# alexeygrigorev/kubernetes-deep-learning

Measured on AMD Instinct MI355X. Metric: images/sec (whole node) + p50 latency, Xception 299x299 at 1/2/4/8 MI355X, higher is better.
Workload: dtype bf16; 1 GPU; model=Keras Xception 299x299 + clothing head (21,067,390 params), global_batch=32, image_size=299, per_gpu_batch=32, parallelism=dp1, ingress=local, egress=local, hipgraph=True, lanes=1, stages=2 (cut after block8_sepconv3)

## Files before the change

kdl/csrc/bindings_gpu.cpp:

```cpp
#include <pybind11/pybind11.h>
#include <pybind11/stl.h>

#include "kernels/launch.h"
#include "runtime/jpeg_huff.h"
#include "runtime/engine.h"
#include "runtime/comm.h"
#include "runtime/dp_hiploop.h"
#include "runtime/hip_backend.h"

namespace py = pybind11;
using namespace kdl;

namespace {

template <typename T>
T* P(const py::dict& d, const char* k) {
  if (!d.contains(k) || d[k].is_none()) return nullptr;
  return reinterpret_cast<T*>(d[k].cast<uintptr_t>());
}
int I(const py::dict& d, const char* k, int def = 0) {
  if (!d.contains(k) || d[k].is_none()) return def;
  return d[k].cast<int>();
}
hipStream_t S(uintptr_t s) { return reinterpret_cast<hipStream_t>(s); }

ConvGemmArgs conv_args(const py::dict& d) {
  ConvGemmArgs a{};
  a.x = P<const uint16_t>(d, "x");
  a.wp = P<const uint16_t>(d, "wp");
  a.bias = P<const float>(d, "bias");
  a.dww = P<const float>(d, "dww");
  a.dwk = P<const uint16_t>(d, "dwk");
  a.res = P<const uint16_t>(d, "res");
  a.y = P<uint16_t>(d, "y");
  a.stamps = P<unsigned long long>(d, "stamps");
  a.B = I(d, "B"); a.H = I(d, "H"); a.W = I(d, "W");
  a.OH = I(d, "OH"); a.OW = I(d, "OW"); a.M = I(d, "M");
  a.ldx = I(d, "ldx"); a.ldy = I(d, "ldy"); a.ldr = I(d, "ldr");
  a.K = I(d, "K"); a.cin = I(d, "cin", 32); a.NF = I(d, "NF");
  a.nstore = I(d, "nstore"); a.stride = I(d, "stride", 1);
  a.relu_in = I(d, "relu_in"); a.relu_out = I(d, "relu_out"); a.opad = I(d, "opad");
  a.dt = I(d, "dt");
  a.krot = I(d, "krot");
  a.ksplit = I(d, "ksplit");
  a.ws = P<float>(d, "ws");
  a.cnt = P<int>(d, "cnt");
  a.ascale = P<const float>(d, "ascale");
  a.ascale_ld = I(d, "ascale_ld");
  return a;
}
float F(const py::dict& d, const char* k, float def) {
  if (!d.contains(k) || d[k].is_none()) return def;
  return d[k].cast<float>();
}
StemArgs stem_args(const py::dict& d) {
  StemArgs a{};
  a.x = P<const void>(d, "x"); a.wp = P<const uint16_t>(d, "wp");
  a.bias = P<const float>(d, "bias"); a.y = P<uint16_t>(d, "y");
  a.B = I(d, "B"); a.H = I(d, "H"); a.W = I(d, "W");
  a.OH = I(d, "OH"); a.OW = I(d, "OW"); a.ldy = I(d, "ldy"); a.in_kind = I(d, "in_kind");
  a.KH = I(d, "KH", 3); a.KW = I(d, "KW", 3); a.stride = I(d, "stride", 2); a.pad = I(d, "pad", 0);
  a.cout = I(d, "cout", 32); a.relu = I(d, "relu", 1); a.dt = I(d, "dt");
  const char* sk[3] = {"scale0", "scale1", "scale2"};
  const char* hk[3] = {"shift0", "shift1", "shift2"};
  for (int c = 0; c < 3; ++c) { a.scale[c] = F(d, sk[c], 1.f); a.shift[c] = F(d, hk[c], 0.f); }
  a.rows = I(d, "rows", 0);
  return a;
}
GapArgs gap_args(const py::dict& d) {
  GapArgs a{};
  a.x = P<const uint16_t>(d, "x"); a.y = P<float>(d, "y"); a.yb = P<uint16_t>(d, "yb");
  a.B = I(d, "B"); a.HW = I(d, "HW"); a.ldx = I(d, "ldx"); a.F = I(d, "F"); a.dt = I(d, "dt");
  return a;
}
FcArgs fc_args(const py::dict& d) {
  FcArgs a{};
  a.x = P<const float>(d, "x"); a.w = P<const float>(d, "w"); a.bias = P<const float>(d, "bias");
  a.out = P<float>(d, "out");
  a.B = I(d, "B"); a.F = I(d, "F"); a.N = I(d, "N"); a.relu = I(d, "relu");
  return a;
}
PatchifyArgs patch_args(const py::dict& d) {
  PatchifyArgs a{};
  a.x = P<const uint8_t>(d, "x"); a.y = P<uint16_t>(d, "y");
  a.B = I(d, "B"); a.H = I(d, "H"); a.W = I(d, "W"); a.P = I(d, "P"); a.ldy = I(d, "ldy");
  const char* sk[3] = {"scale0", "scale1", "scale2"};
  const char* hk[3] = {"shift0", "shift1", "shift2"};
  for (int c = 0; c < 3; ++c) { a.scale[c] = F(d, sk[c], 1.f); a.shift[c] = F(d, hk[c], 0.f); }
  return a;
}
EmbedArgs embed_args(const py::dict& d) {
  EmbedArgs a{};
  a.x = P<uint16_t>(d, "x"); a.cls = P<const float>(d, "cls"); a.pos = P<const float>(d, "pos");
  a.B = I(d, "B"); a.T = I(d, "T"); a.D = I(d, "D");
  return a;
}
LnArgs ln_args(const py::dict& d) {
  LnArgs a{};
  a.x = P<const uint16_t>(d, "x"); a.y = P<uint16_t>(d, "y");
  a.gamma = P<const float>(d, "gamma"); a.beta = P<const float>(d, "beta");
  a.y8 = P<uint8_t>(d, "y8"); a.inv_scale = F(d, "inv_scale", 1.f);
  a.rows = d["rows"].cast<long>(); a.D = I(d, "D"); a.ldx = I(d, "ldx"); a.ldy = I(d, "ldy");
  a.eps = F(d, "eps", 1e-6f);
  return a;
}
AttnArgs attn_args(const py::dict& d) {
  AttnArgs a{};
  a.qkv = P<const uint16_t>(d, "qkv"); a.out = P<uint16_t>(d, "out");
  a.out8 = P<uint8_t>(d, "out8"); a.inv_scale = F(d, "inv_scale", 1.f);
  a.B = I(d, "B"); a.T = I(d, "T"); a.H = I(d, "H"); a.dh = I(d, "dh", 64);
  a.scale = F(d, "scale", 0.125f);
  return a;
}
DwkArgs dwk_args(const py::dict& d) {
  DwkArgs a{};
  a.x = P<const uint16_t>(d, "x"); a.w = P<const float>(d, "w"); a.bias = P<const float>(d, "bias");
  a.y = P<uint16_t>(d, "y"); a.pool = P<float>(d, "pool"); a.w1 = P<const float>(d, "w1");
  a.B = I(d, "B"); a.H = I(d, "H"); a.W = I(d, "W"); a.C = I(d, "C"); a.OH = I(d, "OH"); a.OW = I(d, "OW");
  a.K = I(d, "K"); a.S = I(d, "S", 1); a.pad = I(d, "pad"); a.act = I(d, "act"); a.Cs = I(d, "Cs");
  a.cg = I(d, "cg", 0); a.rb = I(d, "rb", 0); a.tw = I(d, "tw", 0); a.seg = I(d, "seg", 0);
  a.lds_kb = I(d, "lds_kb", 0); a.algo = I(d, "algo", 0); a.pd = I(d, "pd", 0);
// ... 98 lines not shown
}
ResampleArgs resample_args(const py::dict& d) {
  ResampleArgs a{};
  a.desc = P<const ResampleDesc>(d, "desc"); a.h_desc = P<const ResampleDesc>(d, "h_desc");
  a.jdesc = P<const JpegDesc>(d, "jdesc"); a.h_jdesc = P<const JpegDesc>(d, "h_jdesc");
  a.planes = P<const uint8_t>(d, "planes"); a.tmp = P<uint8_t>(d, "tmp"); a.out = P<uint8_t>(d, "out");
  a.plane_cap = U64(d, "plane_cap"); a.tmp_cap = U64(d, "tmp_cap");
  a.n_jdesc = I(d, "n_jdesc"); a.n = I(d, "n"); a.out_rows = I(d, "out_rows");
  a.OH = I(d, "OH"); a.OW = I(d, "OW");
  return a;
}

DwArgs dw_args(const py::dict& d) {
  DwArgs a{};
  a.x = P<const uint16_t>(d, "x"); a.w = P<const float>(d, "w"); a.y = P<uint16_t>(d, "y");
  a.B = I(d, "B"); a.H = I(d, "H"); a.W = I(d, "W"); a.C = I(d, "C"); a.relu_in = I(d, "relu_in");
  a.cg = d.contains("cg") ? I(d, "cg") : 0; a.rb = d.contains("rb") ? I(d, "rb") : 0;
  a.tw = d.contains("tw") ? I(d, "tw") : 0; a.seg = d.contains("seg") ? I(d, "seg") : 0;
  a.algo = d.contains("algo") ? I(d, "algo") : 0; a.pd = d.contains("pd") ? I(d, "pd") : 0;
  return a;
}

void chk(hipError_t e, const char* what) { check_hip(e, what); }

}

PYBIND11_MODULE(_C, m) {
  m.doc() = "kdl MI355X (gfx950) HIP kernels and native executor";

  m.def("conv_gemm", [](int mode, int cfg, py::dict d, uintptr_t s) {
    const auto a = conv_args(d);
    py::gil_scoped_release nogil;
    chk(conv_gemm(mode, cfg, a, S(s)), "conv_gemm");
  });
  m.def("conv_gemm_config", [](int cfg) {
    int bm = 0, bn = 0, th = 0;
    if (conv_gemm_config(cfg, &bm, &bn, &th) != 0) throw std::out_of_range("bad conv_gemm config");
    return py::make_tuple(bm, bn, th);
  });
  m.def("conv_gemm_num_configs", &conv_gemm_num_configs);
  m.def("memcpy_async", [](uintptr_t dst, uintptr_t src, size_t n, int kind, uintptr_t s) {
    py::gil_scoped_release nogil;
    chk(hipMemcpyAsync((void*)dst, (const void*)src, n, (hipMemcpyKind)kind, S(s)), "memcpy_async");
  });
  m.def("dw3x3", [](py::dict d, uintptr_t s) {
    const auto a = dw_args(d);
    py::gil_scoped_release nogil;
    chk(dw3x3(a, S(s)), "dw3x3");
  });
  m.def("stem_conv", [](py::dict d, uintptr_t s) {
    const auto a = stem_args(d);
    py::gil_scoped_release nogil;
    chk(stem_conv(a, S(s)), "stem_conv");
  });
  m.def("pool_add", [](py::dict d, uintptr_t s) {
    const auto a = pool_args(d);
    py::gil_scoped_release nogil;
    chk(pool_add(a, S(s)), "pool_add");
  });
  m.def("head_dense", [](py::dict d, uintptr_t s) {
    const auto a = head_args(d);
    py::gil_scoped_release nogil;
    chk(head_dense(a, S(s)), "head_dense");
  });
  m.def("gap", [](py::dict d, uintptr_t s) {
    const auto a = gap_args(d);
    py::gil_scoped_release nogil;
    chk(gap(a, S(s)), "gap");
  });
  m.def("fc", [](py::dict d, uintptr_t s) {
    const auto a = fc_args(d);
    py::gil_scoped_release nogil;
    chk(fc(a, S(s)), "fc");
  });
  m.def("patchify", [](py::dict d, uintptr_t s) {
    const auto a = patch_args(d);
    py::gil_scoped_release nogil;
    chk(patchify(a, S(s)), "patchify");
  });
  m.def("embed_tokens", [](py::dict d, uintptr_t s) {
    const auto a = embed_args(d);
    py::gil_scoped_release nogil;
    chk(embed_tokens(a, S(s)), "embed_tokens");
  });
  m.def("layernorm", [](py::dict d, uintptr_t s) {
    const auto a = ln_args(d);
    py::gil_scoped_release nogil;
    chk(layernorm(a, S(s)), "layernorm");
  });
  m.def("attention", [](py::dict d, uintptr_t s) {
    const auto a = attn_args(d);
    py::gil_scoped_release nogil;
    chk(attention(a, S(s)), "attention");
  });
  m.def("dwk", [](py::dict d, uintptr_t s) {
    const auto a = dwk_args(d);
    py::gil_scoped_release nogil;
    chk(dwk(a, S(s)), "dwk");
  });
  m.def("dwk_tiles", [](py::dict d) {
    const auto a = dwk_args(d);
    int cg, rb, tw, nt;
    dwk_tiles(a, &cg, &rb, &tw, &nt);
    return py::make_tuple(cg, rb, tw, nt, dwk_seg(a));
  });
  m.def("squeeze_excite", [](py::dict d, uintptr_t s) {
// ... 194 lines not shown
  py::class_<HLLeader>(m, "HipLoopDpLeader")
      .def(py::init([](HipExecBackend* be, loop::Comm* sc, loop::Comm* ga, std::vector<int> buckets, double timeout_s,
                       double ping_s) {
             auto h = new HLLeader();
             h->local = std::make_unique<HipLoopLocal>(be);
             h->lead = std::make_unique<HipLoopDpLeader>(h->local.get(), sc, ga, std::move(buckets), timeout_s, ping_s);
             return h;
           }),
           py::arg("local"), py::arg("scatter"), py::arg("gather"), py::arg("rank_buckets"), py::arg("timeout_s") = 120.0,
           py::arg("ping_s") = 0.0, py::keep_alive<1, 2>(), py::keep_alive<1, 3>(), py::keep_alive<1, 4>())
      .def("api_ptr", [](const HLLeader& l) { return reinterpret_cast<uintptr_t>(l.lead->api()); })
      .def_property_readonly("world", [](const HLLeader& l) { return l.lead->world(); })
      .def_property_readonly("steps", [](const HLLeader& l) { return l.lead->steps(); })
      .def_property_readonly("broken", [](const HLLeader& l) { return l.lead->broken(); })
      .def("send_ctrl", [](HLLeader& l, int cmd, int version) {
        py::gil_scoped_release nogil;
        return l.lead->send_ctrl(cmd, version);
      })
      .def("ping", [](HLLeader& l) {
        py::gil_scoped_release nogil;
        return l.lead->ping();
      });
  py::class_<HLFollower>(m, "HipLoopDpFollower")
      .def(py::init([](HipExecBackend* be, loop::Comm* sc, loop::Comm* ga) {
             auto h = new HLFollower();
             h->local = std::make_unique<HipLoopLocal>(be);
             h->f = std::make_unique<HipLoopDpFollower>(h->local.get(), sc, ga);
             return h;
           }),
           py::keep_alive<1, 2>(), py::keep_alive<1, 3>(), py::keep_alive<1, 4>())
      .def_property_readonly("steps", [](const HLFollower& f) { return f.f->steps(); })
      .def("run", [](HLFollower& f, double liveness_s) {
        DpCtrl c{};
        {
          py::gil_scoped_release nogil;
          c = f.f->run(liveness_s);
        }
        return std::make_tuple(c.cmd, c.version, c.seq);
      }, py::arg("liveness_s") = 30.0);
  m.attr("DP_STOP") = int(DP_STOP);
  m.attr("DP_BATCH") = int(DP_BATCH);
  m.attr("DP_RELOAD") = int(DP_RELOAD);
  m.attr("DP_PING") = int(DP_PING);

  py::class_<Program>(m, "Program")
      .def(py::init<>())
      .def("add_conv_gemm", [](Program& p, const std::string& name, int mode, int cfg, py::dict d) {
        Op op; op.kind = OP_CONV_GEMM; op.name = name; op.mode = mode; op.cfg = cfg; op.g = conv_args(d);
        p.add(op);
      })
      .def("add_stem", [](Program& p, const std::string& name, py::dict d) {
        Op op; op.kind = OP_STEM; op.name = name; op.st = stem_args(d); p.add(op);
      })
      .def("add_pool_add", [](Program& p, const std::string& name, py::dict d) {
        Op op; op.kind = OP_POOL_ADD; op.name = name; op.pa = pool_args(d); p.add(op);
      })
      .def("add_head", [](Program& p, const std::string& name, py::dict d) {
        Op op; op.kind = OP_HEAD; op.name = name; op.hd = head_args(d); p.add(op);
      })
      .def("add_gap", [](Program& p, const std::string& name, py::dict d) {
        Op op; op.kind = OP_GAP; op.name = name; op.gp = gap_args(d); p.add(op);
      })
      .def("add_fc", [](Program& p, const std::string& name, py::dict d) {
        Op op; op.kind = OP_FC; op.name = name; op.fc = fc_args(d); p.add(op);
      })
      .def("add_patchify", [](Program& p, const std::string& name, py::dict d) {
        Op op; op.kind = OP_PATCHIFY; op.name = name; op.pt = patch_args(d); p.add(op);
      })
      .def("add_embed", [](Program& p, const std::string& name, py::dict d) {
        Op op; op.kind = OP_EMBED; op.name = name; op.em = embed_args(d); p.add(op);
      })
      .def("add_layernorm", [](Program& p, const std::string& name, py::dict d) {
        Op op; op.kind = OP_LN; op.name = name; op.ln = ln_args(d); p.add(op);
      })
      .def("add_attention", [](Program& p, const std::string& name, py::dict d) {
        Op op; op.kind = OP_ATTN; op.name = name; op.at = attn_args(d); p.add(op);
      })
      .def("add_dwk", [](Program& p, const std::string& name, py::dict d) {
        Op op; op.kind = OP_DWK; op.name = name; op.dk = dwk_args(d); p.add(op);
      })
      .def("add_se", [](Program& p, const std::string& name, py::dict d) {
        Op op; op.kind = OP_SE; op.name = name; op.se = se_args(d); p.add(op);
      })
      .def("add_chscale", [](Program& p, const std::string& name, py::dict d) {
        Op op; op.kind = OP_CHSCALE; op.name = name; op.cs = chs_args(d); p.add(op);
      })
      .def("add_entry_block", [](Program& p, const std::string& name, int cfg, py::dict d) {
        Op op; op.kind = OP_ENTRY_BLOCK; op.name = name; op.cfg = cfg; op.eb = eb_args(d); p.add(op);
      })
      .def("add_gemm_f8", [](Program& p, const std::string& name, int cfg, py::dict d) {
        Op op; op.kind = OP_GEMM_F8; op.name = name; op.cfg = cfg; op.f8 = f8_args(d); p.add(op);
      })
      .def("add_fc_mfma", [](Program& p, const std::string& name, py::dict d) {
        Op op; op.kind = OP_FC_MFMA; op.name = name; op.fcm = fcm_args(d); p.add(op);
      })
      .def("add_resize", [](Program& p, const std::string& name, py::dict d) {
        Op op; op.kind = OP_RESIZE; op.name = name; op.rs = resize_args(d); p.add(op);
      })
      .def("add_dw", [](Program& p, const std::string& name, py::dict d) {
        Op op; op.kind = OP_DW; op.name = name; op.dw = dw_args(d); p.add(op);
      })
      .def("add_memset", [](Program& p, const std::string& name, uintptr_t ptr, size_t bytes) {
        Op op; op.kind = OP_MEMSET; op.name = name; op.mem_ptr = reinterpret_cast<void*>(ptr);
        op.mem_bytes = bytes; p.add(op);
      })
      .def("set_cfg", [](Program& p, size_t i, int cfg) { p.mutable_op(i).cfg = cfg; })
// ... 18 lines not shown
```

kdl/csrc/kernels/launch.h:

```cpp
#pragma once
#include <hip/hip_runtime.h>
#include <stdint.h>

namespace kdl {

struct ConvGemmArgs {
  const uint16_t* x;
  const uint16_t* wp;
  const float* bias;
  const float* dww;
  const uint16_t* dwk;
  const uint16_t* res;
  uint16_t* y;
  int B, H, W;
  int OH, OW;
  int M;
  int ldx, ldy, ldr;
  int K;
  int cin;
  int NF;
  int nstore;
  int stride;
  int relu_in;
  int relu_out;
// ... 29 lines not shown
  const uint16_t* wr;
  const float* br;
  int B, H, W, OH, OW, ldx, ldy;
  int grid;
  const int4* steps;
  const int* step_off;
  unsigned long long* stamps;
};
hipError_t entry_block(int cfg, const EntryBlockArgs& a, hipStream_t s);
int entry_block_config(int cfg, int* c0, int* c1, int* pc, int* lds, int* occ);

constexpr int C3_CFG_BASE = 208;
hipError_t conv3x3_2d(int cfg, const ConvGemmArgs& a, hipStream_t s);
int conv3x3_2d_config(int cfg, int* bm, int* bn, int* threads);
constexpr int S2D_CFG_BASE = 160;
hipError_t sepconv_2d(int cfg, const ConvGemmArgs& a, hipStream_t s);
int sepconv_2d_config(int cfg, int* bm, int* bn, int* threads);
constexpr int STREAM_CFG_BASE = 3000;
hipError_t gemm_stream(const ConvGemmArgs& a, bool nt, hipStream_t s);
bool gemm_stream_shape(int K, int nstore, int dt = 0);
hipError_t conv_gemm(int mode, int cfg, const ConvGemmArgs& a, hipStream_t s);
hipError_t gemm_pipe(int mode, int cfg, const ConvGemmArgs& a, hipStream_t s);
int gemm_pipe_config(int cfg, int* bm, int* bn, int* threads);
int conv_gemm_config(int cfg, int* bm, int* bn, int* threads);
int conv_gemm_num_configs();

struct DwArgs {
  const uint16_t* x;
  const float* w;
  uint16_t* y;
  int B, H, W, C;
  int relu_in;
  int cg, rb, tw, seg;
  int algo;
  int pd;
};
hipError_t dw3x3(const DwArgs& a, hipStream_t s);

struct StemArgs {
  const void* x;
  const uint16_t* wp;
  const float* bias;
  uint16_t* y;
  int B, H, W, OH, OW, ldy;
  int in_kind;
  int KH, KW, stride, pad, cout;
  float scale[3], shift[3];
  int relu;
  int dt;
  int rows;
};
hipError_t stem_conv(const StemArgs& a, hipStream_t s);

struct PoolAddArgs {
  const uint16_t* x;
  const uint16_t* res;
  uint16_t* y;
  int B, H, W, OH, OW, C;
  int pad_top, pad_left;
  int dt;
  int algo;
  int seg, rb;
};
hipError_t pool_add(const PoolAddArgs& a, hipStream_t s);

struct GapArgs {
  const uint16_t* x;
  float* y;
  uint16_t* yb;
  int B, HW, ldx, F;
  int dt;
};
hipError_t gap(const GapArgs& a, hipStream_t s);

struct FcArgs {
  const float* x;
  const float* w;
  const float* bias;
  float* out;
  int B, F, N, relu;
};
hipError_t fc(const FcArgs& a, hipStream_t s);

struct FcMfmaArgs {
  const uint16_t* xb;
  const uint16_t* wp;
  const float* bias;
  float* out;
  int B, F, N, NF, relu;
  int dt;
};
hipError_t fc_mfma(const FcMfmaArgs& a, hipStream_t s);

struct PatchifyArgs {
  const uint8_t* x;
  uint16_t* y;
  int B, H, W, P, ldy;
  float scale[3], shift[3];
};
hipError_t patchify(const PatchifyArgs& a, hipStream_t s);

struct EmbedArgs {
  uint16_t* x;
  const float* cls;
  const float* pos;
  int B, T, D;
// ... 149 lines not shown
```

kdl/csrc/runtime/engine.cpp:

```cpp
#include "engine.h"

#include <algorithm>

namespace kdl {

void check_hip(hipError_t e, const std::string& what) {
  if (e != hipSuccess) throw std::runtime_error(what + ": " + hipGetErrorString(e));
}

hipError_t run_op(const Op& op, hipStream_t s) {
  switch (op.kind) {
    case OP_CONV_GEMM: return conv_gemm(op.mode, op.cfg, op.g, s);
    case OP_STEM: return stem_conv(op.st, s);
    case OP_POOL_ADD: return pool_add(op.pa, s);
    case OP_HEAD: return head_dense(op.hd, s);
    case OP_RESIZE: return resize_nearest_u8(op.rs, s);
    case OP_MEMSET: return hipMemsetAsync(op.mem_ptr, 0, op.mem_bytes, s);
    case OP_DW: return dw3x3(op.dw, s);
    case OP_GAP: return gap(op.gp, s);
    case OP_FC: return fc(op.fc, s);
    case OP_FC_MFMA: return fc_mfma(op.fcm, s);
    case OP_PATCHIFY: return patchify(op.pt, s);
    case OP_EMBED: return embed_tokens(op.em, s);
    case OP_LN: return layernorm(op.ln, s);
    case OP_ATTN: return attention(op.at, s);
    case OP_DWK: return dwk(op.dk, s);
    case OP_SE: return squeeze_excite(op.se, s);
    case OP_CHSCALE: return channel_scale(op.cs, s);
    case OP_GEMM_F8: return gemm_f8(op.cfg, op.f8, s);
    case OP_ENTRY_BLOCK: return entry_block(op.cfg, op.eb, s);
  }
  return hipErrorInvalidValue;
}

Program::~Program() { reset(); }

void Program::reset() {
  if (exec_) (void)hipGraphExecDestroy(exec_);
  if (graph_) (void)hipGraphDestroy(graph_);
  exec_ = nullptr;
  graph_ = nullptr;
}

void Program::run(hipStream_t s) const {
  for (const auto& op : ops_) check_hip(run_op(op, s), "launch " + op.name);
}

void Program::capture(hipStream_t s) {
  reset();
  check_hip(hipStreamBeginCapture(s, hipStreamCaptureModeThreadLocal), "hipStreamBeginCapture");
  hipError_t err = hipSuccess;
  std::string bad;
  for (const auto& op : ops_) {
    err = run_op(op, s);
    if (err != hipSuccess) { bad = op.name; break; }
  }
  hipGraph_t g = nullptr;
  const hipError_t e2 = hipStreamEndCapture(s, &g);
  if (err != hipSuccess) {
    if (g) (void)hipGraphDestroy(g);
    check_hip(err, "capture launch " + bad);
  }
  check_hip(e2, "hipStreamEndCapture");
  graph_ = g;
  check_hip(hipGraphInstantiate(&exec_, graph_, nullptr, nullptr, 0), "hipGraphInstantiate");
}

void Program::launch(hipStream_t s) const {
  if (exec_) check_hip(hipGraphLaunch(exec_, s), "hipGraphLaunch");
  else run(s);
}

std::vector<float> Program::profile(hipStream_t s, int iters) const {
  const size_t n = ops_.size();
  std::vector<hipEvent_t> ev(n + 1);
  for (auto& e : ev) check_hip(hipEventCreate(&e), "hipEventCreate");
  std::vector<std::vector<float>> t(n);
  for (int it = 0; it < iters; ++it) {
    check_hip(hipEventRecord(ev[0], s), "record");
    for (size_t i = 0; i < n; ++i) {
      check_hip(run_op(ops_[i], s), "launch " + ops_[i].name);
      check_hip(hipEventRecord(ev[i + 1], s), "record");
    }
// ... 20 lines not shown
```

kdl/csrc/runtime/engine.h:

```cpp
#pragma once
#include <hip/hip_runtime.h>

#include <stdexcept>
#include <string>
#include <vector>

#include "../kernels/launch.h"

namespace kdl {

enum OpKind { OP_CONV_GEMM = 0, OP_STEM = 1, OP_POOL_ADD = 2, OP_HEAD = 3, OP_RESIZE = 4, OP_MEMSET = 5, OP_DW = 6, OP_GAP = 7, OP_FC = 8, OP_FC_MFMA = 9,
              OP_PATCHIFY = 10, OP_EMBED = 11, OP_LN = 12, OP_ATTN = 13,
              OP_DWK = 14, OP_SE = 15, OP_CHSCALE = 16, OP_GEMM_F8 = 17,
              OP_ENTRY_BLOCK = 21 };

struct Op {
  OpKind kind;
  std::string name;
  int mode = 0, cfg = 0;
  ConvGemmArgs g{};
  StemArgs st{};
  PoolAddArgs pa{};
  HeadArgs hd{};
  ResizeArgs rs{};
  DwArgs dw{};
  GapArgs gp{};
  FcArgs fc{};
  FcMfmaArgs fcm{};
  PatchifyArgs pt{};
  EmbedArgs em{};
  LnArgs ln{};
  AttnArgs at{};
  DwkArgs dk{};
  SeArgs se{};
  ChScaleArgs cs{};
  GemmF8Args f8{};
  EntryBlockArgs eb{};
  void* mem_ptr = nullptr;
  size_t mem_bytes = 0;
};

void check_hip(hipError_t e, const std::string& what);

hipError_t run_op(const Op& op, hipStream_t s);

class Program {
 public:
  Program() = default;
  ~Program();
  Program(const Program&) = delete;
  Program& operator=(const Program&) = delete;

  void add(const Op& op) {
    if (exec_) throw std::runtime_error("Program already captured; reset() first");
    ops_.push_back(op);
  }
  size_t size() const { return ops_.size(); }
  const Op& op(size_t i) const { return ops_.at(i); }
  Op& mutable_op(size_t i) { return ops_.at(i); }

  void run(hipStream_t s) const;
  void capture(hipStream_t s);
  void launch(hipStream_t s) const;
  bool captured() const { return exec_ != nullptr; }
  void reset();
  std::vector<float> profile(hipStream_t s, int iters) const;

 private:
  std::vector<Op> ops_;
  hipGraph_t graph_ = nullptr;
  hipGraphExec_t exec_ = nullptr;
};

}
```

kdl/engine/xception.py:

```python
from __future__ import annotations

import os
from pathlib import Path

import torch

from ..models import xception as X
from ..models.layers import tf_same_pad
from ..ops import _lib
from ..ops.conv import MODE_CONV, MODE_DW, MODE_PW, ConvGemmLayer, Geometry, conv_weights_nk
from ..ops.pack import bn_scale_shift, pack_fragments, round_up, rowrun_weights
from .base import EngineBase, Step


class XceptionEngine(EngineBase):
    model_name = "xception"

    def __init__(self, params: dict, max_batch: int = 32, device: str | torch.device = "cuda",
                 in_kind: str = "u8", head: X.Head = X.DEFAULT_HEAD, buckets=None,
                 tune_file: str | Path | None = None):
        super().__init__(device, max_batch, buckets)
        self.in_kind = in_kind
        self.head = head
        eb = os.environ.get("KDL_ENTRY_BLOCK", "2:15,3")
        spec = "2,3" if eb == "1" else ("" if eb == "0" else eb)
        self.fused_blocks = {}
        for v in filter(None, (x.strip() for x in spec.split(","))):
            blk, _, cfg = v.partition(":")
            self.fused_blocks[int(blk)] = int(cfg) if cfg else None
        self.size = X.INPUT_SIZE
        self.shapes: dict[str, tuple[int, int, int]] = {}
        self._build(params)
        self._alloc()
        if tune_file and Path(tune_file).exists():
            self.load_tuning(tune_file)

    def _build(self, p: dict) -> None:
        dev = self.device
        S = self.size
        st = X.SPEC
        c1 = st[0].main[0]
        s, t = bn_scale_shift(p, c1.bn)
        w = p[f"{c1.name}/kernel"].double().reshape(27, 32).t() * s[:, None]
        if self.in_kind == "u8":
            bias = t - w.sum(1)
            w = w / 127.5
        else:
            bias = t
        oh1 = (S - 3) // 2 + 1
        self.stem_rows = self.in_kind == "u8" and os.environ.get("KDL_STEM_ROWS", "1") != "0"
        if self.stem_rows:
            self.stem_wp = pack_fragments(rowrun_weights(w, 3, 9, 16), 2, 2).to(dev).contiguous()
        else:
            self.stem_wp = pack_fragments(w, 2, 1).to(dev).contiguous()
        self.stem_bias = bias.float().to(dev)
        self.steps.append(Step("stem", c1.name, src="input", dst="stem1", geom=(S, S, oh1, oh1)))
        self.shapes["stem1"] = (oh1, oh1, 32)
        c2 = st[0].main[1]
        s, t = bn_scale_shift(p, c2.bn)
        w = conv_weights_nk(p[f"{c2.name}/kernel"], 32) * s[:, None]
        lay = ConvGemmLayer(c2.name, MODE_CONV, w, t, cin_pad=32, n=64, relu_out=True, device=dev)
        h = oh1 - 2
        self.steps.append(Step("conv", c2.name, lay, "stem1", "stem2", geom=(oh1, oh1, h, h)))
        self.shapes["stem2"] = (h, h, 64)
        cur, H = "stem2", h
        for bi, blk in enumerate(st[1:], start=1):
            if blk.kind in ("entry", "exit"):
                rc = blk.res_conv
                oh = (H - 1) // 2 + 1
                rname = f"{rc.name}_out"
                lay = self._pw(p, rc, dev)
                _, pt, _ = tf_same_pad(H, 3, 2)
                out = f"block{bi + 1}_out"
                if bi + 1 in self.fused_blocks:
                    from ..ops.entry_block import EntryBlock
                    s1, s2 = (self._sep(p, op, dev) for op in blk.main)
                    g = os.environ.get("KDL_ENTRY_GRID")
                    fb = EntryBlock(f"block{bi + 1}", s1, s2, lay, cfg=self.fused_blocks[bi + 1], device=dev,
                                    grid=int(g) if g else None)
                    self.steps.append(Step("block", f"block{bi + 1}", src=cur, dst=out, geom=(H, H, oh, oh),
                                           extra=dict(eb=fb)))
                    self.shapes[out] = (oh, oh, s2.ldy)
                    cur, H = out, oh
                    continue
                self.steps.append(Step("conv", rc.name, lay, cur, rname, geom=(H, H, oh, oh)))
                self.shapes[rname] = (oh, oh, lay.ldy)
                y = cur
                for op in blk.main:
                    lay = self._sep(p, op, dev)
                    dst = f"{op.name}_out"
                    self.steps.append(Step("conv", op.name, lay, y, dst, geom=(H, H, H, H)))
                    self.shapes[dst] = (H, H, lay.ldy)
                    y = dst
                C = self.shapes[y][2]
                self.steps.append(Step("pool", f"block{bi + 1}_pool", src=y, dst=out, res=rname,
                                       geom=(H, H, oh, oh), extra=dict(pad=pt, C=C)))
                self.shapes[out] = (oh, oh, C)
                cur, H = out, oh
            elif blk.kind == "middle":
                y = cur
                for k, op in enumerate(blk.main):
                    lay = self._sep(p, op, dev)
                    dst = f"{op.name}_out"
                    res = cur if k == len(blk.main) - 1 else None
                    self.steps.append(Step("conv", op.name, lay, y, dst, res=res, geom=(H, H, H, H)))
                    self.shapes[dst] = (H, H, lay.ldy)
                    y = dst
                cur = y
            else:
                for op in blk.main:
                    lay = self._sep(p, op, dev)
                    dst = f"{op.name}_out"
                    self.steps.append(Step("conv", op.name, lay, cur, dst, geom=(H, H, H, H)))
                    self.shapes[dst] = (H, H, lay.ldy)
                    cur = dst
        hd = self.head
# ... 15 lines not shown
            if (a.kind == "conv" and b.kind == "conv" and b.src == a.dst and uses.get(a.dst) == 1
                    and a.res is None and a.layer.relu_out == 0 and b.layer.mode == MODE_DW and b.layer.relu_in):
                a.layer.relu_out, b.layer.relu_in = 1, False

    @staticmethod
    def _pw(p, rc, dev) -> ConvGemmLayer:
        s, t = bn_scale_shift(p, rc.bn)
        cin_pad = round_up(rc.cin, 32)
        w = torch.zeros(rc.cout, cin_pad, dtype=torch.float64)
        w[:, :rc.cin] = p[f"{rc.name}/kernel"].double()[0, 0].t() * s[:, None]
        return ConvGemmLayer(rc.name, MODE_PW, w, t, cin_pad=cin_pad, n=rc.cout, stride=2, device=dev)

    @staticmethod
    def _sep(p, op, dev) -> ConvGemmLayer:
        s, t = bn_scale_shift(p, op.bn)
        cin_pad = round_up(op.cin, 32)
        w = torch.zeros(op.cout, cin_pad, dtype=torch.float64)
        w[:, :op.cin] = p[f"{op.name}/pointwise_kernel"].double()[0, 0].t() * s[:, None]
        dww = torch.zeros(9, cin_pad, dtype=torch.float32)
        dww[:, :op.cin] = p[f"{op.name}/depthwise_kernel"].float()[:, :, :, 0].reshape(9, op.cin)
        return ConvGemmLayer(op.name, MODE_DW, w, t, cin_pad=cin_pad, n=op.cout, dww=dww,
                             relu_in=op.relu_in, relu_out=op.relu_out, device=dev,
                             ksplit=(2, 3, 4) if op.cout >= 1536 else ())

    def _alloc(self) -> None:
        B, S, dev = self.max_batch, self.size, self.device
        if self.in_kind == "u8":
            self.inp = torch.zeros((B, S, S, 3), dtype=torch.uint8, device=dev)
        else:
            self.inp = torch.zeros((B, S, S, 3), dtype=torch.float32, device=dev)
        self.bufs: dict[str, torch.Tensor] = {}
        for name, (h, w, c) in self.shapes.items():
            self.bufs[name] = torch.zeros(B * h * w * c, dtype=torch.bfloat16, device=dev)
        self.logits = torch.zeros((B, self.head.classes), dtype=torch.float32, device=dev)
        self.head_feat = torch.zeros((B, self.head.features), dtype=torch.float32, device=dev)
        self.head_hid = torch.zeros((self.head.features // 64, B, self.head.hidden_units), dtype=torch.float32,
                                    device=dev)
        n = 1
        for st in self.conv_steps():
            if st.layer.mode == MODE_DW:
                H, W, _, _ = st.geom
                n = max(n, B * H * W * st.layer.cin_pad)
        self.dwtmp = torch.zeros(n, dtype=torch.bfloat16, device=dev)
        self.bufs["__dwtmp"] = self.dwtmp

    def _ptr(self, name: str) -> int:
        if name == "input":
            return self.input_ptr()
        if name == "logits":
            return self.output_ptr()
        return _lib.ptr(self.bufs[self._remap.get(name, name)])


    def scratch_buffers(self) -> list[str]:
        return ["__dwtmp"]

    def _emit(self, prog, step: Step, b: int) -> None:
        H, W, OH, OW = step.geom
        if step.kind == "stem":
            prog.add_stem(step.name, dict(x=self.input_ptr(), wp=_lib.ptr(self.stem_wp),
                                          bias=_lib.ptr(self.stem_bias), y=self._ptr(step.dst),
                                          B=b, H=H, W=W, OH=OH, OW=OW, ldy=32,
                                          in_kind=0 if self.in_kind == "u8" else 1, rows=int(self.stem_rows)))
        elif step.kind == "conv":
            self._emit_conv(prog, step, b)
        elif step.kind == "pool":
            prog.add_pool_add(step.name, dict(x=self._ptr(step.src), res=self._ptr(step.res),
                                              y=self._ptr(step.dst), B=b, H=H, W=W, OH=OH, OW=OW,
                                              C=step.extra["C"], pad_top=step.extra["pad"],
                                              pad_left=step.extra["pad"]))
        elif step.kind == "block":
            step.extra["eb"].emit(prog, self._ptr(step.src), self._ptr(step.dst), b, H, W)
        elif step.kind == "head":
            hd = self.head
            prog.add_head(step.name, dict(x=self._ptr(step.src), w1=_lib.ptr(self.w1),
                                          b1=_lib.ptr(self.b1), w2=_lib.ptr(self.w2),
                                          b2=_lib.ptr(self.b2), out=self._ptr("logits"),
                                          feat=_lib.ptr(self.head_feat), hid=_lib.ptr(self.head_hid),
                                          B=b, HW=H * W, ldx=self.shapes[step.src][2],
                                          F=hd.features, H1=hd.hidden_units, NC=hd.classes))

    def _emit_conv(self, prog, step: Step, b: int, split=None, cfg=None) -> None:
        H, W, OH, OW = step.geom
        step.layer.emit(prog, self._ptr(step.src), self._ptr(step.dst), Geometry(b, H, W, OH, OW),
                        res=self._ptr(step.res) if step.res else None, ldx=self.shapes[step.src][2],
                        ldr=self.shapes[step.res][2] if step.res else None, tmp=self._ptr("__dwtmp"),
                        split=split, cfg=cfg)

    def flops_per_image(self) -> float:
        return 2 * 8.356e9
```

Measured before the change: 25640 images/s.

## Fuse Xception stem conv1 and conv2 into one warp-specialized kernel

Adds a fused stem kernel. Producer waves compute the first 3x3 stride-2 conv from uint8 input with MFMA and write halo tiles into an LDS ring, and consumer waves run the second 3x3 conv from LDS and store the 64-channel output. This removes the round trip of the 32-channel stem1 activation through global memory and one kernel launch. The cost is that the halo pixels of conv1 are recomputed per tile, and the design depends on the producer and consumer waves staying balanced. It is enabled by default when stem_rows is set, and the config can be tuned.

```diff
diff --git a/kdl/csrc/bindings_gpu.cpp b/kdl/csrc/bindings_gpu.cpp
--- a/kdl/csrc/bindings_gpu.cpp
+++ b/kdl/csrc/bindings_gpu.cpp
@@ -67,6 +67,15 @@
   a.rows = I(d, "rows", 0);
   return a;
 }
+StemConvArgs stem_conv_args(const py::dict& d) {
+  StemConvArgs a{};
+  a.x = P<const uint8_t>(d, "x"); a.wp1 = P<const uint16_t>(d, "wp1"); a.b1 = P<const float>(d, "b1");
+  a.wp2 = P<const uint16_t>(d, "wp2"); a.b2 = P<const float>(d, "b2"); a.y = P<uint16_t>(d, "y");
+  a.B = I(d, "B"); a.H = I(d, "H"); a.W = I(d, "W"); a.H1 = I(d, "H1"); a.W1 = I(d, "W1");
+  a.OH = I(d, "OH"); a.OW = I(d, "OW"); a.ldy = I(d, "ldy"); a.NF = I(d, "NF"); a.nstore = I(d, "nstore");
+  a.relu_out = I(d, "relu_out"); a.grid = I(d, "grid");
+  return a;
+}
 GapArgs gap_args(const py::dict& d) {
   GapArgs a{};
   a.x = P<const uint16_t>(d, "x"); a.y = P<float>(d, "y"); a.yb = P<uint16_t>(d, "yb");
@@ -271,6 +280,16 @@
     const auto a = stem_args(d);
     py::gil_scoped_release nogil;
     chk(stem_conv(a, S(s)), "stem_conv");
+  });
+  m.def("stem_conv3x3", [](int cfg, py::dict d, uintptr_t s) {
+    const auto a = stem_conv_args(d);
+    py::gil_scoped_release nogil;
+    chk(stem_conv3x3(cfg, a, S(s)), "stem_conv3x3");
+  });
+  m.def("stem_conv3x3_config", [](int cfg) {
+    int bm = 0, bn = 0, th = 0;
+    if (stem_conv3x3_config(cfg, &bm, &bn, &th) != 0) throw std::out_of_range("bad stem_conv3x3 config");
+    return py::make_tuple(bm, bn, th);
   });
   m.def("pool_add", [](py::dict d, uintptr_t s) {
     const auto a = pool_args(d);
@@ -571,6 +590,9 @@
       .def("add_stem", [](Program& p, const std::string& name, py::dict d) {
         Op op; op.kind = OP_STEM; op.name = name; op.st = stem_args(d); p.add(op);
       })
+      .def("add_stem_conv", [](Program& p, const std::string& name, int cfg, py::dict d) {
+        Op op; op.kind = OP_STEM_CONV; op.name = name; op.cfg = cfg; op.sc = stem_conv_args(d); p.add(op);
+      })
       .def("add_pool_add", [](Program& p, const std::string& name, py::dict d) {
         Op op; op.kind = OP_POOL_ADD; op.name = name; op.pa = pool_args(d); p.add(op);
       })
diff --git a/kdl/csrc/kernels/launch.h b/kdl/csrc/kernels/launch.h
--- a/kdl/csrc/kernels/launch.h
+++ b/kdl/csrc/kernels/launch.h
@@ -105,6 +105,23 @@
 };
 hipError_t stem_conv(const StemArgs& a, hipStream_t s);
 
+struct StemConvArgs {
+  const uint8_t* x;
+  const uint16_t* wp1;
+  const float* b1;
+  const uint16_t* wp2;
+  const float* b2;
+  uint16_t* y;
+  int B, H, W;
+  int H1, W1;
+  int OH, OW;
+  int ldy, NF, nstore;
+  int relu_out;
+  int grid;
+};
+hipError_t stem_conv3x3(int cfg, const StemConvArgs& a, hipStream_t s);
+int stem_conv3x3_config(int cfg, int* bm, int* bn, int* threads);
+
 struct PoolAddArgs {
   const uint16_t* x;
   const uint16_t* res;
diff --git a/kdl/csrc/kernels/stem_conv3x3.hip b/kdl/csrc/kernels/stem_conv3x3.hip
--- /dev/null
+++ b/kdl/csrc/kernels/stem_conv3x3.hip
@@ -0,0 +1,283 @@
+#include "common.h"
+#include "launch.h"
+
+#include <algorithm>
+
+namespace kdl {
+
+template <int FM, int FN, int WGM, int WGN, int STAGES, int TH, int TW, int NP>
+__global__ __launch_bounds__(64 * (WGM * WGN + NP)) void stem_conv3x3_kernel(StemConvArgs a) {
+  constexpr int NW = WGM * WGN;
+  constexpr int BM = 16 * FM * WGM;
+  static_assert(BM == TH * TW && TW % 16 == 0, "the M tile is TH x TW pixels, 16-pixel row segments");
+  static_assert(STAGES >= 2 && NP >= 1, "ring depth; producer waves");
+  constexpr int PW = TW + 2, PS = (TH + 2) * PW;
+  constexpr int IPP = (PS + 63) / 64;
+  constexpr int PL = IPP * 1024;
+  constexpr int STAGE = 4 * PL;
+  constexpr int NFRAG = (PS + 15) / 16;
+  constexpr int FPP = (NFRAG + NP - 1) / NP;
+  constexpr int L = STAGES - 1;
+  extern __shared__ __attribute__((aligned(16))) uint8_t smem[];
+  uint8_t* const ring = smem;
+
+  const int tid = threadIdx.x, lane = tid & 63;
+  const int wave = __builtin_amdgcn_readfirstlane(tid >> 6);
+  const int OH = a.OH, OW = a.OW;
+  const int ntw = (OW + TW - 1) / TW, nth = (OH + TH - 1) / TH;
+  const int ntiles = a.B * nth * ntw;
+  const int G = gridDim.x;
+  const int t0 = xcd_remap(blockIdx.x, G);
+  const int Q = t0 < ntiles ? (ntiles - t0 + G - 1) / G : 0;
+  if (Q == 0) return;
+  const int p16 = lane & 15, quad = lane >> 4;
+
+  if (wave >= NW) {
+    const int pw = wave - NW;
+    const int H = a.H, W = a.W, H1 = a.H1, W1 = a.W1;
+    const long total = (long)a.B * H * W * 3, img = (long)H * W * 3;
+    s16x8 bw[2][2];
+    float4 bv[2];
+#pragma unroll
+    for (int j = 0; j < 2; ++j) {
+#pragma unroll
+      for (int ks = 0; ks < 2; ++ks) bw[j][ks] = *(const s16x8*)(a.wp1 + ((j * 2 + ks) * 64 + lane) * 8);
+      bv[j] = *(const float4*)(a.b1 + 16 * j + 4 * quad);
+    }
+#pragma unroll
+    for (int j = 0; j < 2; ++j)
+      asm volatile("" ::"v"(bw[j][0]), "v"(bw[j][1]), "v"(bv[j].x), "v"(bv[j].y), "v"(bv[j].z), "v"(bv[j].w));
+    const int rq = 8 * (quad & 1);
+    const int W6 = 6 * W;
+    const int lane_off = rq + (quad >> 1) * 3 * W;
+    const uint32_t m0 = rq ? 0xffu : ~0u, m1 = rq ? 0u : ~0u;
+    const bool row2 = quad < 2;
+    int pr[FPP], pc[FPP], lo[FPP];
+#pragma unroll
+    for (int i = 0; i < FPP; ++i) {
+      const int s = (pw + i * NP) * 16 + p16;
+      const int sc = min(s, PS - 1);
+      pr[i] = sc / PW;
+      pc[i] = sc - pr[i] * PW;
+      lo[i] = (quad >> 1) * PL + s * 16 + (quad & 1) * 8;
+    }
+    typedef uint32_t u32x3 __attribute__((ext_vector_type(3)));
+    typedef u32x3 u32x3_a4 __attribute__((aligned(4)));
+    u32x3 d[FPP][2];
+    int tt[FPP][2];
+    const uint8_t* xb = a.x;
+    int rem = 0;
+    auto load = [&](int tq) {
+      const int tile = t0 + tq * G;
+      const int bimg = tile / (nth * ntw), trem = tile - bimg * (nth * ntw);
+      const int h0 = (trem / ntw) * TH, w0 = (trem % ntw) * TW;
+      const long sbase = bimg * img;
+      const uintptr_t ia = (uintptr_t)a.x + sbase;
+      const int sb_lo = (int)(ia & 3);
+      xb = (const uint8_t*)(ia - sb_lo);
+      rem = (int)std::min(total - sbase + sb_lo, (long)0x7fffffff);
+      const int last = (rem - 12) & ~3;
+#pragma unroll
+      for (int i = 0; i < FPP; ++i) {
+        if (pw + i * NP >= NFRAG) continue;
+        const int r = min(h0 + pr[i], H1 - 1), c = min(w0 + pc[i], W1 - 1);
+        const int t0b = r * W6 + c * 6 + lane_off + sb_lo;
+#pragma unroll
+        for (int ks = 0; ks < 2; ++ks) {
+          const int t = t0b + (ks == 1 && row2 ? W6 : 0);
+          const int al = t & ~3;
+          const bool over = al + 12 > rem;
+          d[i][ks] = *(const u32x3_a4*)(xb + (over ? last : al));
+          tt[i][ks] = over ? (t | (int)0x80000000) : t;
+        }
+      }
+    };
+    auto build = [&](int slotbuf, int next) {
+      uint8_t* base = ring + slotbuf * STAGE;
+      uint32_t w[FPP][2][2];
+#pragma unroll
+      for (int i = 0; i < FPP; ++i) {
+        if (pw + i * NP >= NFRAG) continue;
+#pragma unroll
+        for (int ks = 0; ks < 2; ++ks) {
+          uint32_t d0 = d[i][ks][0], d1 = d[i][ks][1], d2 = d[i][ks][2];
+          const int t = tt[i][ks] & 0x7fffffff;
+          uint32_t sh = t & 3;
+          if (tt[i][ks] < 0) {
+            uint32_t w0b = 0u, w1b = 0u;
+#pragma unroll
+            for (int j = 0; j < 8; ++j) {
+              const uint32_t v = t + j < rem ? xb[t + j] : 0u;
+              if (j < 4) w0b |= v << (8 * j); else w1b |= v << (8 * (j - 4));
+            }
+            d0 = w0b; d1 = w1b; d2 = 0u; sh = 0u;
+          }
+          const uint32_t k0 = ks == 0 || row2 ? m0 : 0u, k1 = ks == 0 || row2 ? m1 : 0u;
+          w[i][ks][0] = __builtin_amdgcn_alignbyte(d1, d0, sh) & k0;
+          w[i][ks][1] = __builtin_amdgcn_alignbyte(d2, d1, sh) & k1;
+        }
+      }
+      if (next >= 0) load(next);
+#pragma unroll
+      for (int i = 0; i < FPP; ++i) {
+        if (pw + i * NP >= NFRAG) continue;
+        f32x4 acc[2] = {(f32x4){0.f, 0.f, 0.f, 0.f}, (f32x4){0.f, 0.f, 0.f, 0.f}};
+#pragma unroll
+        for (int ks = 0; ks < 2; ++ks) {
+          u32x4 pk;
+#pragma unroll
+          for (int j = 0; j < 4; ++j) {
+            const uint32_t wd = w[i][ks][j >> 1];
+            pk[j] = pack_bf16((float)((wd >> (16 * (j & 1))) & 0xffu), (float)((wd >> (16 * (j & 1) + 8)) & 0xffu));
+          }
+          const s16x8 af = __builtin_bit_cast(s16x8, pk);
+#pragma unroll
+          for (int j = 0; j < 2; ++j) acc[j] = mfma16(bw[j][ks], af, acc[j]);
+        }
+#pragma unroll
+        for (int j = 0; j < 2; ++j) {
+          const float v0 = fmaxf(acc[j][0] + bv[j].x, 0.f), v1 = fmaxf(acc[j][1] + bv[j].y, 0.f);
+          const float v2 = fmaxf(acc[j][2] + bv[j].z, 0.f), v3 = fmaxf(acc[j][3] + bv[j].w, 0.f);
+          *(u32x2*)(base + 2 * j * PL + lo[i]) = (u32x2){pack_bf16(v0, v1), pack_bf16(v2, v3)};
+        }
+      }
+    };
+    load(0);
+    for (int p = 0; p < L; ++p)
+      if (p < Q) build(p, p + 1 < Q ? p + 1 : -1);
+    for (int q = 0; q < Q; ++q) {
+      asm volatile("s_waitcnt lgkmcnt(0)\n\ts_barrier" ::: "memory");
+      if (q + L < Q) build((q + L) % STAGES, q + L + 1 < Q ? q + L + 1 : -1);
+    }
+    return;
+  }
+
+  const int wm = wave / WGN, wn = wave % WGN;
+  s16x8 bw[9][FN];
+#pragma unroll
+  for (int t = 0; t < 9; ++t)
+#pragma unroll
+    for (int j = 0; j < FN; ++j)
+      bw[t][j] = *(const s16x8*)(a.wp2 + (((long)(wn * FN + j) * 9 + t) * 64 + lane) * 8);
+  const int kb = quad, col = p16;
+  float4 bvr[FN];
+#pragma unroll
+  for (int j = 0; j < FN; ++j) bvr[j] = *(const float4*)(a.b2 + wn * FN * 16 + j * 16 + 4 * quad);
+  int aoff[FM], prow[FM], pcol[FM];
+#pragma unroll
+  for (int i = 0; i < FM; ++i) {
+    const int pix = (wm * FM + i) * 16 + p16;
+    const int r = pix / TW, c = pix - r * TW;
+    aoff[i] = kb * PL + (r * PW + c) * 16;
+    const int op = (wm * FM + i) * 16 + col;
+    prow[i] = op / TW;
+    pcol[i] = op - prow[i] * TW;
+  }
+  asm volatile("s_waitcnt vmcnt(0)" ::: "memory");
+
+  for (int q = 0; q < Q; ++q) {
+    asm volatile("s_waitcnt lgkmcnt(0)\n\ts_barrier" ::: "memory");
+    const uint8_t* pb = ring + (q % STAGES) * STAGE;
+    f32x4 acc[FM][FN];
+#pragma unroll
+    for (int i = 0; i < FM; ++i)
+#pragma unroll
+      for (int j = 0; j < FN; ++j) acc[i][j] = (f32x4){0.f, 0.f, 0.f, 0.f};
+#pragma unroll
+    for (int t = 0; t < 9; ++t) {
+      const int toff = ((t / 3) * PW + t % 3) * 16;
+      s16x8 af[FM];
+#pragma unroll
+      for (int i = 0; i < FM; ++i) af[i] = *(const s16x8*)(pb + aoff[i] + toff);
+#pragma unroll
+      for (int i = 0; i < FM; ++i)
+#pragma unroll
+        for (int j = 0; j < FN; ++j) acc[i][j] = mfma16(bw[t][j], af[i], acc[i][j]);
+    }
+    const int tile = t0 + q * G;
+    const int bimg = tile / (nth * ntw), trem = tile - bimg * (nth * ntw);
+    const int h0 = (trem / ntw) * TH, w0 = (trem % ntw) * TW;
+#pragma unroll
+    for (int i = 0; i < FM; ++i) {
+      const int h = h0 + prow[i], w = w0 + pcol[i];
+      if (h < OH && w < OW) {
+        uint16_t* yrow = a.y + ((long)(bimg * OH + h) * OW + w) * a.ldy;
+#pragma unroll
+        for (int j = 0; j < FN; ++j) {
+          const int n = wn * FN * 16 + j * 16 + 4 * quad;
+          float v0 = acc[i][j][0] + bvr[j].x, v1 = acc[i][j][1] + bvr[j].y;
+          float v2 = acc[i][j][2] + bvr[j].z, v3 = acc[i][j][3] + bvr[j].w;
+          if (a.relu_out == 1) {
+            v0 = fmaxf(v0, 0.f); v1 = fmaxf(v1, 0.f); v2 = fmaxf(v2, 0.f); v3 = fmaxf(v3, 0.f);
+          }
+          if (n < a.nstore) *(u32x2*)(yrow + n) = (u32x2){pack_bf16(v0, v1), pack_bf16(v2, v3)};
+        }
+      }
+    }
+  }
+  asm volatile("s_waitcnt vmcnt(0)" ::: "memory");
+}
+
+#define KDL_SC3_CONFIGS(X)            \
+  X(0, 2, 4, 4, 1, 2, 8, 16, 4)       \
+  X(1, 2, 4, 4, 1, 2, 8, 16, 2)       \
+  X(2, 2, 4, 4, 1, 3, 8, 16, 4)       \
+  X(3, 2, 4, 4, 1, 3, 8, 16, 2)
+
+static int sc3_num_cus() {
+  static int n = 0;
+  if (n == 0) {
+    int dev = 0;
+    if (hipGetDevice(&dev) != hipSuccess || hipDeviceGetAttribute(&n, hipDeviceAttributeMultiprocessorCount, dev) != hipSuccess || n <= 0)
+      n = 256;
+  }
+  return n;
+}
+
+template <int FM, int FN, int WGM, int WGN, int ST, int TH, int TW, int NP>
+static hipError_t launch_sc3(const StemConvArgs& a, hipStream_t s) {
+  constexpr int BN = 16 * FN * WGN, NT = 64 * (WGM * WGN + NP);
+  if (!a.x || !a.wp1 || !a.b1 || !a.wp2 || !a.b2 || !a.y || a.B <= 0 || a.H < 7 || a.W < 7 ||
+      a.H1 != (a.H - 3) / 2 + 1 || a.W1 != (a.W - 3) / 2 + 1 || a.OH != a.H1 - 2 || a.OW != a.W1 - 2 ||
+      a.NF * 16 != BN || a.nstore <= 0 || a.nstore > a.ldy || a.nstore % 4 || a.ldy % 4 || a.relu_out < 0 ||
+      a.relu_out > 1 || a.grid < 0 || (long)a.B * a.OH * a.OW > 0x7fffffffL ||
+      (long)a.H * a.W * 3 > (1L << 30))
+    return hipErrorInvalidValue;
+  constexpr int PS = (TH + 2) * (TW + 2), IPP = (PS + 63) / 64;
+  const size_t smem = (size_t)ST * 4 * IPP * 1024;
+  const int ntiles = a.B * ((a.OH + TH - 1) / TH) * ((a.OW + TW - 1) / TW);
+  static int per_cu = 0;
+  if (per_cu == 0) {
+    int n = 0;
+    if (hipOccupancyMaxActiveBlocksPerMultiprocessor(&n, stem_conv3x3_kernel<FM, FN, WGM, WGN, ST, TH, TW, NP>, NT,
+                                                     smem) != hipSuccess || n <= 0)
+      n = 1;
+    per_cu = n;
+  }
+  int grid = std::min(ntiles, sc3_num_cus() * per_cu);
+  if (a.grid > 0) grid = std::min(grid, a.grid);
+  hipLaunchKernelGGL((stem_conv3x3_kernel<FM, FN, WGM, WGN, ST, TH, TW, NP>), dim3(grid), dim3(NT), smem, s, a);
+  return hipGetLastError();
+}
+
+int stem_conv3x3_config(int cfg, int* bm, int* bn, int* threads) {
+  switch (cfg) {
+#define KDL_SC3INFO(id, fm, fn, wgm, wgn, st, th, tw, np) \
+  case id: *bm = 16 * fm * wgm; *bn = 16 * fn * wgn; *threads = 64 * (wgm * wgn + np); return 0;
+    KDL_SC3_CONFIGS(KDL_SC3INFO)
+#undef KDL_SC3INFO
+    default: return -1;
+  }
+}
+
+hipError_t stem_conv3x3(int cfg, const StemConvArgs& a, hipStream_t s) {
+  switch (cfg) {
+#define KDL_SC3CASE(id, fm, fn, wgm, wgn, st, th, tw, np) \
+  case id: return launch_sc3<fm, fn, wgm, wgn, st, th, tw, np>(a, s);
+    KDL_SC3_CONFIGS(KDL_SC3CASE)
+#undef KDL_SC3CASE
+    default: return hipErrorInvalidValue;
+  }
+}
+
+}
diff --git a/kdl/csrc/runtime/engine.cpp b/kdl/csrc/runtime/engine.cpp
--- a/kdl/csrc/runtime/engine.cpp
+++ b/kdl/csrc/runtime/engine.cpp
@@ -29,6 +29,7 @@
     case OP_CHSCALE: return channel_scale(op.cs, s);
     case OP_GEMM_F8: return gemm_f8(op.cfg, op.f8, s);
     case OP_ENTRY_BLOCK: return entry_block(op.cfg, op.eb, s);
+    case OP_STEM_CONV: return stem_conv3x3(op.cfg, op.sc, s);
   }
   return hipErrorInvalidValue;
 }
diff --git a/kdl/csrc/runtime/engine.h b/kdl/csrc/runtime/engine.h
--- a/kdl/csrc/runtime/engine.h
+++ b/kdl/csrc/runtime/engine.h
@@ -12,7 +12,7 @@
 enum OpKind { OP_CONV_GEMM = 0, OP_STEM = 1, OP_POOL_ADD = 2, OP_HEAD = 3, OP_RESIZE = 4, OP_MEMSET = 5, OP_DW = 6, OP_GAP = 7, OP_FC = 8, OP_FC_MFMA = 9,
               OP_PATCHIFY = 10, OP_EMBED = 11, OP_LN = 12, OP_ATTN = 13,
               OP_DWK = 14, OP_SE = 15, OP_CHSCALE = 16, OP_GEMM_F8 = 17,
-              OP_ENTRY_BLOCK = 21 };
+              OP_ENTRY_BLOCK = 21, OP_STEM_CONV = 22 };
 
 struct Op {
   OpKind kind;
@@ -36,6 +36,7 @@
   ChScaleArgs cs{};
   GemmF8Args f8{};
   EntryBlockArgs eb{};
+  StemConvArgs sc{};
   void* mem_ptr = nullptr;
   size_t mem_bytes = 0;
 };
diff --git a/kdl/engine/xception.py b/kdl/engine/xception.py
--- a/kdl/engine/xception.py
+++ b/kdl/engine/xception.py
@@ -11,6 +11,10 @@
 from ..ops.conv import MODE_CONV, MODE_DW, MODE_PW, ConvGemmLayer, Geometry, conv_weights_nk
 from ..ops.pack import bn_scale_shift, pack_fragments, round_up, rowrun_weights
 from .base import EngineBase, Step
+
+
+STEM_FUSED_NAME = "block1_stem_conv"
+STEM_FUSED_CONFIGS = 4
 
 
 class XceptionEngine(EngineBase):
@@ -54,14 +58,20 @@
         else:
             self.stem_wp = pack_fragments(w, 2, 1).to(dev).contiguous()
         self.stem_bias = bias.float().to(dev)
-        self.steps.append(Step("stem", c1.name, src="input", dst="stem1", geom=(S, S, oh1, oh1)))
-        self.shapes["stem1"] = (oh1, oh1, 32)
         c2 = st[0].main[1]
         s, t = bn_scale_shift(p, c2.bn)
         w = conv_weights_nk(p[f"{c2.name}/kernel"], 32) * s[:, None]
         lay = ConvGemmLayer(c2.name, MODE_CONV, w, t, cin_pad=32, n=64, relu_out=True, device=dev)
         h = oh1 - 2
-        self.steps.append(Step("conv", c2.name, lay, "stem1", "stem2", geom=(oh1, oh1, h, h)))
+        self.stem_fused = self.stem_rows and os.environ.get("KDL_STEM_FUSED", "1") != "0"
+        self.stem_fused_cfg = int(os.environ.get("KDL_STEM_FUSED_CFG", "0"))
+        if self.stem_fused:
+            self.steps.append(Step("stemconv", STEM_FUSED_NAME, lay, "input", "stem2", geom=(S, S, h, h),
+                                   extra=dict(h1=oh1)))
+        else:
+            self.steps.append(Step("stem", c1.name, src="input", dst="stem1", geom=(S, S, oh1, oh1)))
+            self.shapes["stem1"] = (oh1, oh1, 32)
+            self.steps.append(Step("conv", c2.name, lay, "stem1", "stem2", geom=(oh1, oh1, h, h)))
         self.shapes["stem2"] = (h, h, 64)
         cur, H = "stem2", h
         for bi, blk in enumerate(st[1:], start=1):
@@ -183,6 +193,12 @@
         return _lib.ptr(self.bufs[self._remap.get(name, name)])
 
 
+    def apply_tuning(self, d: dict) -> None:
+        v = d.get(STEM_FUSED_NAME)
+        if isinstance(v, int) and 0 <= v < STEM_FUSED_CONFIGS and "KDL_STEM_FUSED_CFG" not in os.environ:
+            self.stem_fused_cfg = v
+        super().apply_tuning(d)
+
     def scratch_buffers(self) -> list[str]:
         return ["__dwtmp"]
 
@@ -193,6 +209,14 @@
                                           bias=_lib.ptr(self.stem_bias), y=self._ptr(step.dst),
                                           B=b, H=H, W=W, OH=OH, OW=OW, ldy=32,
                                           in_kind=0 if self.in_kind == "u8" else 1, rows=int(self.stem_rows)))
+        elif step.kind == "stemconv":
+            lay, h1 = step.layer, step.extra["h1"]
+            assert lay.nf_max == 4 and lay.ldy == 64, "stem_conv3x3 holds all 64 outputs in one N tile"
+            prog.add_stem_conv(step.name, self.stem_fused_cfg,
+                               dict(x=self.input_ptr(), wp1=_lib.ptr(self.stem_wp), b1=_lib.ptr(self.stem_bias),
+                                    wp2=_lib.ptr(lay.wp), b2=_lib.ptr(lay.bias), y=self._ptr(step.dst),
+                                    B=b, H=H, W=W, H1=h1, W1=h1, OH=OH, OW=OW, ldy=lay.ldy, NF=lay.nf_max,
+                                    nstore=lay.ldy, relu_out=int(lay.relu_out)))
         elif step.kind == "conv":
             self._emit_conv(prog, step, b)
         elif step.kind == "pool":
```

Measured after the change: 25940 images/s, median of 6. 1.2% higher.
